# ucuapps/OpenGlue

Hardware: NVIDIA H100
Metric: image-pairs/sec at N=M=2048, d=256, 9 GNN layers, 100 Sinkhorn iters (higher is better)
Workload: dtype fp16x3 (fp16 hi/lo operands with power-of-two tensor scales, 3 products, fp32 accumulate)

## Files before the change

openglue_b200/csrc/sinkhorn.cuh:

```cuda
#pragma once
#include "common.cuh"
#include "tc_common.cuh"
#include <math_constants.h>
#include <algorithm>

namespace og {

struct SinkArgs {
  static constexpr bool kBackward = false;
  const float* S; int64_t lds, strideS;
  const float* dustbin;
  int B, n, m, iters;
  float reg;
  float norm, log_a_last, log_b_last;
  float* scores;
  float* u;
  float* partial;
  unsigned int* barrier;
  int SP, rows_per_strip, mpad;
  float* hist_u;
  float* hist_v;
};

constexpr int SINK_WARPS = 8;
constexpr int64_t SINK_BARRIER_BYTES = 256 * 128;
constexpr int SINK_MAX_COLS = 8192;
constexpr int SINK_MAX_STRIPS = 32;
constexpr float LOG2E_F = 1.4426950408889634f;

__device__ __forceinline__ void grid_barrier(unsigned int* counter, unsigned int target) {
  __syncthreads();
  if (threadIdx.x == 0) {
    __threadfence();
    atomicAdd(counter, 1u);
    unsigned int seen;
    do {
      asm volatile("ld.acquire.gpu.global.u32 %0, [%1];" : "=r"(seen) : "l"(counter) : "memory");
    } while (seen < target);
    __threadfence();
  }
  __syncthreads();
}

typedef unsigned long long f32x2;
__device__ __forceinline__ f32x2 pk2(float x, float y) { f32x2 r; asm("mov.b64 %0, {%1, %2};" : "=l"(r) : "f"(x), "f"(y)); return r; }
__device__ __forceinline__ void upk2(f32x2 v, float& x, float& y) { asm("mov.b64 {%0, %1}, %2;" : "=f"(x), "=f"(y) : "l"(v)); }
#define OG_F32X2_OP(name, expr)                                        \
  __device__ __forceinline__ f32x2 name(f32x2 a, f32x2 b) {            \
    float ax, ay, bx, by; upk2(a, ax, ay); upk2(b, bx, by);            \
    auto op = [](float u, float v) { return expr; };                   \
    return pk2(op(ax, bx), op(ay, by));                                \
  }
OG_F32X2_OP(add2, __fadd_rn(u, v))
OG_F32X2_OP(sub2, __fsub_rn(u, v))
OG_F32X2_OP(mul2, __fmul_rn(u, v))
#undef OG_F32X2_OP
__device__ __forceinline__ f32x2 fma2(f32x2 a, f32x2 b, f32x2 c) {
  float ax, ay, bx, by, cx, cy; upk2(a, ax, ay); upk2(b, bx, by); upk2(c, cx, cy);
  return pk2(__fmaf_rn(ax, bx, cx), __fmaf_rn(ay, by, cy));
}

template <int V, int W>
struct SinkStrip {
  static constexpr int C = 128 * V, MC = W * C, G = SINK_WARPS / W;
  int b, strip, tid, lane, grp, sub, c0, r0, r1;
  template <class Args>
  __device__ __forceinline__ explicit SinkStrip(const Args& a) {
    b = blockIdx.x / a.SP; strip = blockIdx.x % a.SP;
    tid = threadIdx.x; lane = tid & 31;
    grp = (tid >> 5) / W; sub = (tid >> 5) % W;
    c0 = sub * C;
    r0 = strip * a.rows_per_strip;
    r1 = min(r0 + a.rows_per_strip, a.n + 1);
  }
};

template <int V, int W, int SLOTS, bool EVICT_FIRST, class Args>
struct SinkRowRing {
  static constexpr int C = 128 * V, G = SINK_WARPS / W;
  float* slot;
// ... 52 lines not shown
      for (int k = 0; k < V; ++k) z[k] = make_float4(dz, dz, dz, dz);
      return;
    }
    if (!bytes) {
#pragma unroll
      for (int k = 0; k < V; ++k) z[k] = make_float4(0.f, 0.f, 0.f, 0.f);
      return;
    }
    const uint32_t sl = consumed % SLOTS, ph = (consumed / SLOTS) & 1;
    while (!tc::mbar_try_wait(&bar[sl], ph)) {}
    const float4* src = reinterpret_cast<const float4*>(slot + sl * C);
    if (full) {
#pragma unroll
      for (int k = 0; k < V; ++k) z[k] = src[lane + 32 * k];
    } else {
#pragma unroll
      for (int k = 0; k < V; ++k) {
        const int idx = lane + 32 * k;
        const int c = c0 + 4 * idx;
        const int m = a.m;
        float4 q = (c < m) ? src[idx] : make_float4(0.f, 0.f, 0.f, 0.f);
        if (c < m && c + 3 >= m) {
          if (c + 1 >= m) q.y = 0.f;
          if (c + 2 >= m) q.z = 0.f;
          q.w = 0.f;
        }
        z[k] = q;
      }
    }
    ++consumed;
    __syncwarp();
    const int nxt = row + SLOTS * G;
    if (lane == 0 && nxt < end_real) copy(sl, nxt);
    if (a.reg != 1.0f) {
      const float reg = a.reg;
#pragma unroll
      for (int k = 0; k < V; ++k) {
        z[k].x = __fdiv_rn(z[k].x, reg); z[k].y = __fdiv_rn(z[k].y, reg);
        z[k].z = __fdiv_rn(z[k].z, reg); z[k].w = __fdiv_rn(z[k].w, reg);
      }
    }
  }
};

template <int V, int W, class X>
__device__ __forceinline__ const X* sink_row_exchange(X* xr, X mine, const SinkStrip<V, W>& s, uint32_t& rowpar) {
  X* x = xr + (rowpar * SinkStrip<V, W>::G + s.grp) * W;
  if (s.lane == 0) x[s.sub] = mine;
  asm volatile("bar.sync %0, %1;" ::"r"(1 + s.grp), "n"(W * 32) : "memory");
  rowpar ^= 1u;
  return x;
}

template <int V, int W, class Args, class Update>
__device__ __forceinline__ void sink_column_reduce(const Args& a, const SinkStrip<V, W>& s, float* red, const float4 (&cacc)[V],
                                                   float cacc_m, int k, Update update) {
  const int m = a.m;
  float* myred = red + s.grp * a.mpad;
#pragma unroll
  for (int q = 0; q < V; ++q) {
    const int c = s.c0 + 4 * (s.lane + 32 * q);
    if (c < m) *reinterpret_cast<float4*>(myred + c) = cacc[q];
  }
  __syncthreads();
  if (s.sub == 0 && s.lane == 0) myred[m] = cacc_m;
  __syncthreads();
  const int64_t buf = (int64_t)(k & 1) * a.B * a.SP + (int64_t)s.b * a.SP;
  float* part = a.partial + (buf + s.strip) * a.mpad;
  for (int j = s.tid; j <= m; j += blockDim.x) {
    float sum = 0.f;
#pragma unroll
    for (int w = 0; w < SinkStrip<V, W>::G; ++w) sum += red[w * a.mpad + j];
    part[j] = sum;
  }
  grid_barrier(a.barrier + 32 * s.b, (unsigned int)(k + 1) * (unsigned int)a.SP);
  const float* pb = a.partial + buf * a.mpad;
  for (int j4 = s.tid; 4 * j4 <= m; j4 += blockDim.x) {
    float4 c = make_float4(0.f, 0.f, 0.f, 0.f);
#pragma unroll 8
    for (int sp = 0; sp < a.SP; ++sp) {
      const float4 q = __ldcg(reinterpret_cast<const float4*>(pb + (int64_t)sp * a.mpad) + j4);
      c.x += q.x; c.y += q.y; c.z += q.z; c.w += q.w;
    }
    const float cc[4] = {c.x, c.y, c.z, c.w};
#pragma unroll
    for (int e = 0; e < 4; ++e) {
      const int j = 4 * j4 + e;
      if (j < m) update(j, cc[e]);
      else if (j == m) update(SinkStrip<V, W>::MC, cc[e]);
    }
  }
  __syncthreads();
}

template <int V, int W, int SLOTS>
__global__ void __launch_bounds__(SINK_WARPS * 32, (V <= 8) ? 2 : 1) sinkhorn_kernel(SinkArgs a) {
  extern __shared__ __align__(128) float og_sink_smem[];
  using Strip = SinkStrip<V, W>;
  constexpr int C = Strip::C, MC = Strip::MC, G = Strip::G;
  float* v_s = og_sink_smem;
  float* red = og_sink_smem + MC + 4;
  float* ring = red + G * a.mpad;
  uint64_t* bars = reinterpret_cast<uint64_t*>(ring + SINK_WARPS * SLOTS * C);
  float2* xr = reinterpret_cast<float2*>(bars + SINK_WARPS * SLOTS);
  const Strip s(a);
  const int n = a.n, m = a.m, c0 = s.c0, lane = s.lane, sub = s.sub;
  const float a_reg = expf(a.norm), a_last = expf(a.log_a_last);
  SinkRowRing<V, W, SLOTS, true, SinkArgs> rows(a, s, ring, bars);
  const float dz = rows.dz;

  for (int j = s.tid; j < MC; j += blockDim.x) v_s[j] = (j < m) ? 0.f : -CUDART_INF_F;
  if (s.tid == 0) v_s[MC] = 0.f;
  __syncthreads();

  rows.prime();
  uint32_t rowpar = 0;
  const f32x2 log2e2 = pk2(LOG2E_F, LOG2E_F);
  for (int it = 0; it < a.iters; ++it) {
    f32x2 cacc[2 * V];
#pragma unroll
    for (int k = 0; k < 2 * V; ++k) cacc[k] = 0ull;
    float cacc_m = 0.f;
    const float v_m = v_s[MC];

    for (int row = s.r0 + s.grp; row < s.r1; row += G) {
      float4 q[V];
      rows.take(row, q);
      f32x2 z[2 * V];
#pragma unroll
      for (int k = 0; k < V; ++k) { z[2 * k] = pk2(q[k].x, q[k].y); z[2 * k + 1] = pk2(q[k].z, q[k].w); }
      const float t_m = dz + v_m;
      float mx = (sub == 0) ? t_m : -CUDART_INF_F;
#pragma unroll
      for (int k = 0; k < V; ++k) {
        const ulonglong2 vv = *reinterpret_cast<const ulonglong2*>(v_s + c0 + 4 * (lane + 32 * k));
        z[2 * k] = add2(z[2 * k], vv.x); z[2 * k + 1] = add2(z[2 * k + 1], vv.y);
// ... 25 lines not shown
        f_w = ex2_approx((mx - mxg) * LOG2E_F);
      }
      const float w_i = __fdiv_rn((row < n) ? a_reg : a_last, s_i) * f_w;
      if ((it == a.iters - 1 || a.hist_u) && sub == 0 && lane == 0) {
        const float u_i = ((row < n) ? a.norm : a.log_a_last) - (mxg + logf(s_i));
        if (it == a.iters - 1) a.u[(int64_t)s.b * (n + 1) + row] = u_i;
        if (a.hist_u) a.hist_u[((int64_t)s.b * a.iters + it) * (n + 1) + row] = u_i;
      }
      const f32x2 w2 = pk2(w_i, w_i);
#pragma unroll
      for (int k = 0; k < 2 * V; ++k) cacc[k] = fma2(z[k], w2, cacc[k]);
      cacc_m = fmaf(e_m, w_i, cacc_m);
    }
    rows.prime();
    float4 c4[V];
#pragma unroll
    for (int k = 0; k < V; ++k) { upk2(cacc[2 * k], c4[k].x, c4[k].y); upk2(cacc[2 * k + 1], c4[k].z, c4[k].w); }
    sink_column_reduce(a, s, red, c4, cacc_m, it, [&](int j, float c) {
      v_s[j] = ((j < MC) ? a.norm : a.log_b_last) + v_s[j] - logf(c);
    });
    if (a.hist_v && s.strip == 0) {
      float* hv = a.hist_v + ((int64_t)s.b * (a.iters + 1) + it + 1) * (m + 1);
      for (int j = s.tid; j <= m; j += blockDim.x) hv[j] = (j < m) ? v_s[j] : v_s[MC];
    }
  }

  {
    const float v_m = v_s[MC];
    for (int row = s.r0 + s.grp; row < s.r1; row += G) {
      float4 z[V];
      rows.take(row, z);
      float u_i = 0.f;
      if (a.iters > 0) {
        if (lane == 0) u_i = __ldcg(a.u + (int64_t)s.b * (n + 1) + row);
        u_i = __shfl_sync(0xffffffffu, u_i, 0);
      }
      float* out = a.scores + ((int64_t)s.b * (n + 1) + row) * (m + 1);
#pragma unroll
      for (int k = 0; k < V; ++k) {
        const int c = c0 + 4 * (lane + 32 * k);
        if (c < m) {
          const float4 vv = *reinterpret_cast<const float4*>(v_s + c);
          if (c + 0 < m) out[c + 0] = (z[k].x + u_i) + vv.x - a.norm;
          if (c + 1 < m) out[c + 1] = (z[k].y + u_i) + vv.y - a.norm;
          if (c + 2 < m) out[c + 2] = (z[k].z + u_i) + vv.z - a.norm;
          if (c + 3 < m) out[c + 3] = (z[k].w + u_i) + vv.w - a.norm;
        }
      }
      if (sub == 0 && lane == 0) out[m] = (dz + u_i) + v_m - a.norm;
    }
  }
}

struct SinkPlan { int V, W, slots, occ, SP, rows_per_strip, mpad, pairs_per_launch; size_t smem; };

constexpr size_t sinkhorn_smem(bool backward, int V, int W, int slots, int mpad) {
  const int C = 128 * V, G = SINK_WARPS / W, vecs = backward ? 3 : 1;
  const size_t xbytes = backward ? sizeof(float) : sizeof(float2);
  return ((size_t)vecs * (W * C + 4) + (size_t)G * mpad + (size_t)SINK_WARPS * slots * C) * sizeof(float) +
         (size_t)SINK_WARPS * slots * sizeof(uint64_t) + (size_t)2 * G * W * xbytes + 128;
}

inline int sinkhorn_plan(bool backward, int B, int n, int m, SinkPlan* p) {
  const char* who = backward ? "sinkhorn_bwd" : "sinkhorn";
  if (m <= 512)                { p->V = 4;  p->W = 1; p->slots = 2; }
  else if (m <= 1024)          { p->V = 4;  p->W = 2; p->slots = 2; }
  else if (m <= 2048)          { p->V = 8;  p->W = 2; p->slots = 2; }
  else if (m <= 4096)          { p->V = 16; p->W = 2; p->slots = backward ? 1 : 2; }
  else if (m <= SINK_MAX_COLS) { p->V = 16; p->W = 4; p->slots = 1; }
  else return fail(OG_EUNSUPPORTED, "%s: m = %d > %d columns not supported (swap the images)", who, m, SINK_MAX_COLS);
  p->mpad = (int)align_up(m + 1, 4);
  p->smem = sinkhorn_smem(backward, p->V, p->W, p->slots, p->mpad);
  p->occ = (p->V <= 8 && 2 * (p->smem + 1024) <= OG_SMEM_OPTIN_MAX) ? 2 : 1;
  const int sms = device_info().ok ? device_info().sm_count : 132;
  const int ctas = sms * p->occ;
  p->pairs_per_launch = std::min(B < ctas ? B : ctas, (int)(SINK_BARRIER_BYTES / 128));
  int sp = std::min(ctas / p->pairs_per_launch, SINK_MAX_STRIPS);
  const int max_sp = cdiv(n + 1, SINK_WARPS / p->W);
  if (sp > max_sp) sp = max_sp;
  if (sp < 1) sp = 1;
  p->SP = sp;
  p->rows_per_strip = cdiv(n + 1, sp);
  return OG_OK;
}

inline int sinkhorn_check_rows(const char* who, const float* S, int64_t lds, int64_t strideS, int m) {
  if (lds % 4 != 0 || lds < m || (reinterpret_cast<uintptr_t>(S) & 15) || strideS % 4 != 0)
    return fail(OG_EINVAL, "%s: S rows must be 16-byte aligned (lds %% 4 == 0, lds >= m)", who);
  return OG_OK;
}

struct SinkConsts { float norm, log_a_last, log_b_last; };
inline SinkConsts sinkhorn_consts(int n, int m) {
  const float norm = -logf((float)(n + m));
  return {norm, norm + (float)log((double)m),
          norm + (float)log((double)n)};
}

template <auto Kernel, int V, int W, int SLOTS, class Args>
inline int sinkhorn_coop_launch(const Args& a, const SinkPlan& p, cudaStream_t stream) {
  constexpr size_t smem_max = sinkhorn_smem(Args::kBackward, V, W, SLOTS, 128 * V * W + 4);
  static_assert(smem_max <= OG_SMEM_OPTIN_MAX, "Sinkhorn kernel: shared memory beyond what one block may opt in to");
  if (const int rc = smem_opt_in<Kernel>((int)smem_max)) return rc;
  cudaLaunchConfig_t cfg = {};
  cfg.gridDim = dim3(a.B * a.SP);
  cfg.blockDim = dim3(SINK_WARPS * 32);
  cfg.dynamicSmemBytes = p.smem;
  cfg.stream = stream;
  cudaLaunchAttribute attr[1];
  attr[0].id = cudaLaunchAttributeCooperative;
  attr[0].val.cooperative = 1;
  cfg.attrs = attr; cfg.numAttrs = 1;
  OG_CUDA(cudaLaunchKernelEx(&cfg, Kernel, a));
  launch_counter()++;
  return OG_OK;
}

template <class Launch>
inline int sinkhorn_for_each_launch(const SinkPlan& p, int B, unsigned int* barrier, cudaStream_t stream, Launch&& launch) {
  for (int b0 = 0; b0 < B; b0 += p.pairs_per_launch) {
    const int nb = std::min(p.pairs_per_launch, B - b0);
    OG_CUDA(cudaMemsetAsync(barrier, 0, (size_t)nb * 128, stream));
    if (const int rc = launch(b0, nb)) return rc;
  }
  return OG_OK;
}

inline int64_t sinkhorn_workspace_bytes(int B, int n, int m) {
  SinkPlan p;
  if (sinkhorn_plan(false, B, n, m, &p) != OG_OK) return -1;
  return SINK_BARRIER_BYTES + align_up((int64_t)B * (n + 1) * 4, 256) + align_up(2LL * B * SINK_MAX_STRIPS * p.mpad * 4, 256);
}

inline int sinkhorn_launch(const float* S, int64_t lds, int64_t strideS, const float* dustbin, int B, int n, int m,
                           int iters, float reg, float* scores, void* ws, int64_t ws_bytes, cudaStream_t stream,
                           float* hist_u = nullptr, float* hist_v = nullptr) {
  SinkPlan p;
  if (const int rc = sinkhorn_plan(false, B, n, m, &p)) return rc;
  if (ws_bytes < sinkhorn_workspace_bytes(B, n, m)) return fail(OG_EWORKSPACE, "sinkhorn: workspace too small");
  if (const int rc = sinkhorn_check_rows("sinkhorn", S, lds, strideS, m)) return rc;
  char* w = static_cast<char*>(ws);
  unsigned int* barrier = reinterpret_cast<unsigned int*>(w); w += SINK_BARRIER_BYTES;
  float* u = reinterpret_cast<float*>(w); w += align_up((int64_t)B * (n + 1) * 4, 256);
  float* partial = reinterpret_cast<float*>(w);
  const SinkConsts k = sinkhorn_consts(n, m);
  if (hist_v) OG_CUDA(cudaMemsetAsync(hist_v, 0, (size_t)B * (iters + 1) * (m + 1) * sizeof(float), stream));
  return sinkhorn_for_each_launch(p, B, barrier, stream, [&](int b0, int nb) {
    SinkArgs a;
    a.S = S + (int64_t)b0 * strideS; a.lds = lds; a.strideS = strideS; a.dustbin = dustbin;
    a.B = nb; a.n = n; a.m = m; a.iters = iters; a.reg = reg;
    a.norm = k.norm; a.log_a_last = k.log_a_last; a.log_b_last = k.log_b_last;
    a.scores = scores + (int64_t)b0 * (n + 1) * (m + 1);
    a.u = u; a.partial = partial; a.barrier = barrier;
    a.SP = p.SP; a.rows_per_strip = p.rows_per_strip; a.mpad = p.mpad;
    a.hist_u = hist_u ? hist_u + (int64_t)b0 * iters * (n + 1) : nullptr;
    a.hist_v = hist_v ? hist_v + (int64_t)b0 * (iters + 1) * (m + 1) : nullptr;
    if (p.V == 4 && p.W == 1) return sinkhorn_coop_launch<sinkhorn_kernel<4, 1, 2>, 4, 1, 2>(a, p, stream);
    if (p.V == 4)             return sinkhorn_coop_launch<sinkhorn_kernel<4, 2, 2>, 4, 2, 2>(a, p, stream);
    if (p.V == 8)             return sinkhorn_coop_launch<sinkhorn_kernel<8, 2, 2>, 8, 2, 2>(a, p, stream);
    if (p.W == 2)             return sinkhorn_coop_launch<sinkhorn_kernel<16, 2, 2>, 16, 2, 2>(a, p, stream);
    return sinkhorn_coop_launch<sinkhorn_kernel<16, 4, 1>, 16, 4, 1>(a, p, stream);
  });
}

}
```

openglue_b200/csrc/sinkhorn_bwd.cuh:

```cuda
#pragma once
#include "sinkhorn.cuh"

namespace og {

struct SinkBwdArgs {
  static constexpr bool kBackward = true;
  const float* S; int64_t lds, strideS;
  const float* dustbin;
  int B, n, m, iters;
  float reg, norm, log_a_last, log_b_last;
  const float* hist_u;
  const float* hist_v;
  const float* ubar_init;
  const float* vbar_init;
  float* hist_coef;
  float* hist_cvec;
  float* hist_vbar;
  float* hist_wq;
  float* partial;
  unsigned int* barrier;
  int SP, rows_per_strip, mpad;
};

template <int V, int W, int SLOTS>
__global__ void __launch_bounds__(SINK_WARPS * 32, (V <= 8) ? 2 : 1) sinkhorn_bwd_kernel(SinkBwdArgs a) {
  extern __shared__ __align__(128) float og_sinkb_smem[];
  using Strip = SinkStrip<V, W>;
  constexpr int C = Strip::C, MC = Strip::MC, G = Strip::G;
  float* cvec_s = og_sinkb_smem;
  float* vbar_s = cvec_s + MC + 4;
  float* wq_s = vbar_s + MC + 4;
  float* red = wq_s + MC + 4;
  float* ring = red + G * a.mpad;
  uint64_t* bars = reinterpret_cast<uint64_t*>(ring + SINK_WARPS * SLOTS * C);
  float* xr = reinterpret_cast<float*>(bars + SINK_WARPS * SLOTS);
  const Strip s(a);
  const int n = a.n, m = a.m, T = a.iters, b = s.b, tid = s.tid;
  const float ia_reg = expf(-a.norm), ia_last = expf(-a.log_a_last);
  SinkRowRing<V, W, SLOTS, false, SinkBwdArgs> rows(a, s, ring, bars);
  const float dz = rows.dz;

  for (int j = tid; j <= MC; j += blockDim.x) {
    float vb = 0.f;
    if (j < m) vb = __ldg(a.vbar_init + (int64_t)b * (m + 1) + j);
    else if (j == MC) vb = __ldg(a.vbar_init + (int64_t)b * (m + 1) + m);
    vbar_s[j] = vb;
  }
  __syncthreads();

  rows.prime();
  uint32_t rowpar = 0;
  for (int it = T - 1; it >= 0; --it) {
    const float* vt = a.hist_v + ((int64_t)b * (T + 1) + it + 1) * (m + 1);
    const float* vtm1 = vt - (m + 1);
    for (int j = tid; j <= MC; j += blockDim.x) {
      float cv = -CUDART_INF_F, wq = 0.f;
      const int jj = (j < m) ? j : (j == MC ? m : -1);
      if (jj >= 0) {
        const float lb = (jj < m) ? a.norm : a.log_b_last;
        cv = __ldcg(vt + jj) - lb;
        wq = expf(__ldcg(vtm1 + jj) - cv);
      }
      cvec_s[j] = cv; wq_s[j] = wq;
    }
    __syncthreads();
    if (s.strip == 0) {
      const int64_t o = ((int64_t)b * T + it) * (m + 1);
      for (int j = tid; j <= m; j += blockDim.x) {
        const int js = (j < m) ? j : MC;
        a.hist_cvec[o + j] = cvec_s[js]; a.hist_vbar[o + j] = vbar_s[js]; a.hist_wq[o + j] = wq_s[js];
      }
    }
    float4 cacc[V];
#pragma unroll
// ... 159 lines not shown

inline int64_t sinkhorn_hist_floats(int B, int n, int m, int T) { return (int64_t)B * T * (n + 1) + (int64_t)B * (T + 1) * (m + 1); }

inline int64_t sinkhorn_bwd_workspace_bytes(int B, int n, int m, int T) {
  SinkPlan p;
  if (sinkhorn_plan(true, B, n, m, &p) != OG_OK) return -1;
  const int64_t nrs = cdiv(n + 1, SINKB_RS_ROWS);
  int64_t f = 0;
  f += align_up((int64_t)B * (n + 1), 64) + align_up((int64_t)B * (m + 1), 64);
  f += align_up((int64_t)B * nrs * (m + 1), 64);
  f += align_up((int64_t)B * T * (n + 1), 64) + 3 * align_up((int64_t)B * T * (m + 1), 64);
  f += align_up(2LL * B * SINK_MAX_STRIPS * p.mpad, 64) + align_up((int64_t)B, 64);
  return SINK_BARRIER_BYTES + 256 + f * 4;
}

inline int sinkhorn_bwd_launch(const float* S, int64_t lds, int64_t strideS, const float* dustbin, int B, int n, int m, int iters, float reg,
                               const float* hist, const float* G, float* dZ, float* ddustbin, void* ws, int64_t ws_bytes,
                               cudaStream_t stream) {
  SinkPlan p;
  if (const int rc = sinkhorn_plan(true, B, n, m, &p)) return rc;
  if (ws_bytes < sinkhorn_bwd_workspace_bytes(B, n, m, iters)) return fail(OG_EWORKSPACE, "sinkhorn_bwd: workspace too small");
  if (const int rc = sinkhorn_check_rows("sinkhorn_bwd", S, lds, strideS, m)) return rc;
  const int T = iters;
  const int64_t nrs = cdiv(n + 1, SINKB_RS_ROWS);
  char* w = static_cast<char*>(ws);
  unsigned int* barrier = reinterpret_cast<unsigned int*>(w); w += SINK_BARRIER_BYTES;
  unsigned int* counter = reinterpret_cast<unsigned int*>(w); w += 256;
  float* f = reinterpret_cast<float*>(w);
  auto take = [&](int64_t nfl) { float* r = f; f += align_up(nfl, 64); return r; };
  float* ubar_init = take((int64_t)B * (n + 1));
  float* vbar_init = take((int64_t)B * (m + 1));
  float* colpart = take((int64_t)B * nrs * (m + 1));
  float* hist_coef = take((int64_t)B * T * (n + 1));
  float* hist_cvec = take((int64_t)B * T * (m + 1));
  float* hist_vbar = take((int64_t)B * T * (m + 1));
  float* hist_wq = take((int64_t)B * T * (m + 1));
  float* partial = take(2LL * B * SINK_MAX_STRIPS * p.mpad);
  float* per_pair = take(B);
  const SinkConsts k = sinkhorn_consts(n, m);
  const int m1 = m + 1, n1 = n + 1;
  sinkb_rowsum_kernel<<<cdiv(B * n1, 8), 256, 0, stream>>>(G, B * n1, m1, ubar_init);
  OG_LAUNCH_CHECK("sinkb_rowsum_kernel");
  sinkb_colsum_kernel<<<dim3(cdiv(m1, 256), (unsigned)nrs, B), 256, 0, stream>>>(G, n1, m1, colpart);
  OG_LAUNCH_CHECK("sinkb_colsum_kernel");
  sinkb_colsum_finish_kernel<<<dim3(cdiv(m1, 256), B), 256, 0, stream>>>(colpart, (int)nrs, m1, vbar_init);
  OG_LAUNCH_CHECK("sinkb_colsum_finish_kernel");
  launch_counter() += 3;
  SinkBwdArgs a;
  a.S = S; a.lds = lds; a.strideS = strideS; a.dustbin = dustbin; a.B = B; a.n = n; a.m = m; a.iters = T; a.reg = reg;
  a.norm = k.norm; a.log_a_last = k.log_a_last; a.log_b_last = k.log_b_last;
  a.hist_u = hist; a.hist_v = hist + (int64_t)B * T * (n + 1);
  a.ubar_init = ubar_init; a.vbar_init = vbar_init;
  a.hist_coef = hist_coef; a.hist_cvec = hist_cvec; a.hist_vbar = hist_vbar; a.hist_wq = hist_wq;
  a.partial = partial; a.barrier = barrier; a.SP = p.SP; a.rows_per_strip = p.rows_per_strip; a.mpad = p.mpad;
  if (T > 0) {
    const int rc = sinkhorn_for_each_launch(p, B, barrier, stream, [&](int b0, int nb) {
      SinkBwdArgs g = a;
      g.B = nb;
      g.S = S + (int64_t)b0 * strideS;
      g.hist_u = a.hist_u + (int64_t)b0 * T * n1; g.hist_v = a.hist_v + (int64_t)b0 * (T + 1) * m1;
      g.ubar_init = ubar_init + (int64_t)b0 * n1; g.vbar_init = vbar_init + (int64_t)b0 * m1;
      g.hist_coef = hist_coef + (int64_t)b0 * T * n1; g.hist_cvec = hist_cvec + (int64_t)b0 * T * m1;
      g.hist_vbar = hist_vbar + (int64_t)b0 * T * m1; g.hist_wq = hist_wq + (int64_t)b0 * T * m1;
      if (p.V == 4 && p.W == 1) return sinkhorn_coop_launch<sinkhorn_bwd_kernel<4, 1, 2>, 4, 1, 2>(g, p, stream);
      if (p.V == 4)             return sinkhorn_coop_launch<sinkhorn_bwd_kernel<4, 2, 2>, 4, 2, 2>(g, p, stream);
      if (p.V == 8)             return sinkhorn_coop_launch<sinkhorn_bwd_kernel<8, 2, 2>, 8, 2, 2>(g, p, stream);
      if (p.W == 2)             return sinkhorn_coop_launch<sinkhorn_bwd_kernel<16, 2, 1>, 16, 2, 1>(g, p, stream);
      return sinkhorn_coop_launch<sinkhorn_bwd_kernel<16, 4, 1>, 16, 4, 1>(g, p, stream);
    });
    if (rc != OG_OK) return rc;
  }
  sinkb_dz_kernel<<<dim3(cdiv(m1, SINKB_TC), cdiv(n1, SINKB_TR), B), 256, 0, stream>>>(a, G, dZ, 1.f / reg);
  OG_LAUNCH_CHECK("sinkb_dz_kernel");
  OG_CUDA(cudaMemsetAsync(counter, 0, 4, stream));
  sinkb_dustbin_kernel<<<B, 256, 0, stream>>>(dZ, B, n, m, per_pair, counter, ddustbin);
  OG_LAUNCH_CHECK("sinkb_dustbin_kernel");
  launch_counter() += 2;
  return OG_OK;
}

}
```

openglue_b200/csrc/linear_sm90.cuh:

```cuda
#pragma once
#include "tc_common.cuh"
#include <algorithm>
#include <type_traits>

namespace og {

struct TcLinearArgs {
  const float* A;  int64_t lda;  int64_t strideA;
  const float* A2; int64_t lda2; int64_t strideA2;
  int k1, k2;
  int b_rows_per_batch;
  const float* bias;
  int rows, nout, batch;
  float alpha;
  int relu;
  const float* R; int64_t ldr; int64_t strideR;
  const float* rscale;
  float* Y;   float* Yhi;  float* Ylo;  int64_t ldy;  int64_t strideY;
  float* Yt;  float* Ythi; float* Ytlo; int64_t ldyt; int64_t strideYt;
};

struct F16LinearArgs {
  const float* A;  int64_t lda;  int64_t strideA;
  const float* A2; int64_t lda2; int64_t strideA2;
// ... 125 lines not shown
      if (*timeout_flag) asm volatile("trap;");
    }
    return;
  }
  setmaxnreg_inc<240>();
  const int c = wg - 1, tid = threadIdx.x & 127, warp = tid >> 5, lane = tid & 31, g = lane >> 2, t = lane & 3;
  const int r0 = c * 64 + warp * 16 + g;

  float s_a = 1.f, amax_a = 0.f;
  if constexpr (F16) {
#pragma unroll
    for (int i = 0; i < 3; ++i) if (a.amax_in[i]) amax_a = fmaxf(amax_a, __ldcg(a.amax_in[i]));
    s_a = f16_scale_for(amax_a);
    if (blockIdx.x == 0 && threadIdx.x == 128) {
      if (a.nkinds > 1) {
        for (int kk = 0; kk < a.nkinds; ++kk) {
          const float* w2 = a.w_meta + 4 * kk;
          const float so = f16_scale_for(fabsf(a.alpha) * fmaf(amax_a, __ldg(w2 + 1), __ldg(w2 + 2)));
          if (a.kind0 + kk == 1 && a.scale_out) *a.scale_out = so;
          if (a.kind0 + kk == 2 && a.scale_out_v) *a.scale_out_v = so;
        }
      } else if (!a.Y && a.scale_out) {
        *a.scale_out = f16_scale_for(fabsf(a.alpha) * fmaf(amax_a, __ldg(a.w_meta + 1), __ldg(a.w_meta + 2)));
      }
    }
  }

  float racc[64], acc[64];
  uint32_t ahi0[4][4], alo0[4][4], ahi1[4][4], alo1[4][4];
  uint32_t it = 0, timed_out = 0;

  auto split_a = [&](uint32_t it_, uint32_t (&ahi)[4][4], uint32_t (&alo)[4][4]) {
    const int s = it_ % S;
    mbar_wait_flag(&full[s], (it_ / S) & 1, timed_out);
    const uint8_t* st = smem + s * C::STAGE;
#pragma unroll
    for (int kk = 0; kk < 4; ++kk) {
      if constexpr (F16) {
        const uint8_t* box = st + (kk >> 1) * BM * 128;
        const int col = (kk & 1) * 16 + 2 * t;
#pragma unroll
        for (int q = 0; q < 4; ++q) {
          const float2 v = *reinterpret_cast<const float2*>(sw128_f32(box, r0 + (q & 1) * 8, col + (q >> 1) * 8));
          split_f16x2(v.x * s_a, v.y * s_a, ahi[kk][q], alo[kk][q]);
          if (a.swap_halves) { ahi[kk][q] = __byte_perm(ahi[kk][q], 0, 0x1032); alo[kk][q] = __byte_perm(alo[kk][q], 0, 0x1032); }
        }
      } else {
#pragma unroll
        for (int q = 0; q < 4; ++q) split_tf32(*sw128_f32(st, r0 + (q & 1) * 8, 8 * kk + t + (q >> 1) * 4), ahi[kk][q], alo[kk][q]);
      }
    }
  };

  if (c == 1) named_bar_arrive(TURN + 0, 256);
#pragma unroll 1
  for (int tile = blockIdx.x; tile < ntiles; tile += gridDim.x) {
    int n0, m0, bz;
    tile_origin(tile, tiles_n, tiles_m, n0, m0, bz);
    const bool last_tile = tile + (int)gridDim.x >= ntiles;
#pragma unroll
    for (int i = 0; i < 64; ++i) racc[i] = 0.f;

    auto mma_block = [&](int kb, const uint32_t (&ahi)[4][4], const uint32_t (&alo)[4][4], uint32_t (&nhi)[4][4],
                         uint32_t (&nlo)[4][4]) {
      const int s = it % S;
      const bool last = last_tile && kb == nkb - 1;
      if (last && timed_out) *timeout_flag = 1;
      const uint32_t bhi = smem_u32(smem + s * C::STAGE + C::A_BYTES), blo = bhi + C::B_TILE;
      named_bar_sync(TURN + c, 256);
      fence_operands(acc);
      wgmma_fence();
#pragma unroll
      for (int kk = 0; kk < 4; ++kk) {
        const uint64_t dhi = make_wgdesc_sw128(bhi + kk * 32), dlo = make_wgdesc_sw128(blo + kk * 32);
        const int acc0 = (kb % C::CHUNK != 0 || kk) ? 1 : 0;
        if constexpr (F16) {
          wgmma_f16_m64n128(acc, alo[kk], dhi, acc0);
          wgmma_f16_m64n128(acc, ahi[kk], dlo, 1);
          wgmma_f16_m64n128(acc, ahi[kk], dhi, 1);
        } else {
          wgmma_tf32_m64n128(acc, alo[kk], dhi, acc0);
          wgmma_tf32_m64n128(acc, ahi[kk], dlo, 1);
          wgmma_tf32_m64n128(acc, ahi[kk], dhi, 1);
        }
      }
      wgmma_commit();
      if (!(last && c == 1)) named_bar_arrive(TURN + (c ^ 1), 256);
      if (kb + 1 < nkb) split_a(it + 1, nhi, nlo);
      wgmma_wait<0>();
      fence_operands(acc);
      if (tid == 0) mbar_arrive(&empty[s]);
      if (kb % C::CHUNK == C::CHUNK - 1 || kb == nkb - 1) {
#pragma unroll
        for (int i = 0; i < 64; ++i) racc[i] += acc[i];
      }
      ++it;
    };
    split_a(it, ahi0, alo0);
#pragma unroll 1
    for (int kb = 0; kb < nkb; kb += 2) {
      mma_block(kb, ahi0, alo0, ahi1, alo1);
      if (kb + 1 < nkb) mma_block(kb + 1, ahi1, alo1, ahi0, alo0);
    }

    if constexpr (F16) {
      const float s_w = __ldg(a.w_meta);
      int okind = a.Y ? 1 : (a.Yh ? 2 : 3), kidx = 0, ocols = a.nout;
      float alpha_t = a.alpha / (s_a * s_w), sos = 1.f;
      const float* wm = a.w_meta;
      if (a.nkinds > 1) {
        kidx = n0 / a.kind_cols; okind = a.kind0 + kidx + 1; ocols = a.kind_cols;
        wm = a.w_meta + 4 * kidx;
        alpha_t = a.alpha / (s_a * __ldg(wm));
      }
      if (okind != 1) sos = f16_scale_for(fabsf(a.alpha) * fmaf(amax_a, __ldg(wm + 1), __ldg(wm + 2)));
      float tmax = 0.f;
      if (okind == 1) {
#pragma unroll
        for (int h = 0; h < 2; ++h) {
          const int grow = m0 + r0 + 8 * h;
          if (grow >= a.rows) continue;
          const float* rrow = a.R ? a.R + (int64_t)bz * a.strideR + (int64_t)grow * a.ldr : nullptr;
#pragma unroll
          for (int jh = 0; jh < 16; jh += 8) {
            float bv[16], rv[16];
#pragma unroll
            for (int i = 0; i < 16; ++i) {
              const int col = n0 + 8 * (jh + (i >> 1)) + 2 * t + (i & 1);
              const bool in = col < a.nout;
              bv[i] = a.bias && in ? __ldg(a.bias + col) : 0.f;
              rv[i] = rrow && in ? rrow[col] : 0.f;
            }
#pragma unroll
            for (int jj = 0; jj < 8; ++jj) {
              const int j = jh + jj;
              const int col = n0 + 8 * j + 2 * t;
              if (col >= a.nout) continue;
              const bool two = col + 1 < a.nout;
              float y0 = fmaf(racc[4 * j + 2 * h], alpha_t, bv[2 * jj]);
              float y1 = two ? fmaf(racc[4 * j + 2 * h + 1], alpha_t, bv[2 * jj + 1]) : 0.f;
              if (a.relu) { y0 = fmaxf(y0, 0.f); y1 = fmaxf(y1, 0.f); }
              const int64_t o = (int64_t)bz * a.strideY + (int64_t)grow * a.ldy + col;
              if (a.R) {
                y0 += rv[2 * jj];
                if (two) y1 += rv[2 * jj + 1];
              }
              if (two) *reinterpret_cast<float2*>(a.Y + o) = make_float2(y0, y1);
              else a.Y[o] = y0;
              tmax = fmaxf(tmax, fmaxf(fabsf(y0), fabsf(y1)));
            }
          }
        }
      } else {
        uint32_t hv[2][16], lv[2][16];
#pragma unroll
        for (int j = 0; j < 16; ++j) {
          const int col = n0 + 8 * j + 2 * t;
          const bool two = col + 1 < a.nout;
          const float b0 = a.bias && col < a.nout ? __ldg(a.bias + col) : 0.f;
          const float b1 = a.bias && two ? __ldg(a.bias + col + 1) : 0.f;
#pragma unroll
          for (int h = 0; h < 2; ++h) {
            float y0 = fmaf(racc[4 * j + 2 * h], alpha_t, b0);
            float y1 = two ? fmaf(racc[4 * j + 2 * h + 1], alpha_t, b1) : 0.f;
            if (a.relu) { y0 = fmaxf(y0, 0.f); y1 = fmaxf(y1, 0.f); }
            split_f16x2(y0 * sos, y1 * sos, hv[h][j], lv[h][j]);
          }
        }
        if (okind == 2) {
          const bool wide = a.ldy % 8 == 0 && a.strideY % 8 == 0 && al16(a.Yh) && al16(a.Yl);
#pragma unroll
          for (int h = 0; h < 2; ++h) {
            const int grow = m0 + r0 + 8 * h;
            const int64_t orow = (int64_t)bz * a.strideY + (int64_t)grow * a.ldy - kidx * ocols;
            if (wide) {
#pragma unroll
              for (int q = 0; q < 4; ++q) {
                const uint4 vh = quad_gather_b16(hv[h], q, t), vl = quad_gather_b16(lv[h], q, t);
                const int col = n0 + 8 * (4 * q + t);
                if (grow >= a.rows || col >= a.nout) continue;
                if (col + 8 <= a.nout) {
                  *reinterpret_cast<uint4*>(a.Yh + orow + col) = vh;
                  *reinterpret_cast<uint4*>(a.Yl + orow + col) = vl;
                } else {
                  store_b16_run(a.Yh + orow + col, vh, a.nout - col);
                  store_b16_run(a.Yl + orow + col, vl, a.nout - col);
                }
              }
            } else if (grow < a.rows) {
#pragma unroll
              for (int j = 0; j < 16; ++j) {
                const int col = n0 + 8 * j + 2 * t;
                if (col >= a.nout) continue;
                store_half_pair(a.Yh + orow + col, hv[h][j], col + 1 < a.nout);
                store_half_pair(a.Yl + orow + col, lv[h][j], col + 1 < a.nout);
              }
            }
          }
        } else {
#pragma unroll
          for (int h = 0; h < 2; ++h) {
            const int grow = m0 + r0 + 8 * h;
            if (grow < a.rows) {
#pragma unroll
              for (int j = 0; j < 16; ++j) {
                const int col = n0 + 8 * j + 2 * t;
// ... 5 lines not shown
                  a.Ytl[o + a.ldyt] = __ushort_as_half((unsigned short)(lv[h][j] >> 16));
                }
              }
            }
          }
        }
      }
      if (okind == 1 && a.amax_out) {
        tmax = warp_max(tmax);
        if (lane == 0 && tmax > 0.f) atomic_amax(a.amax_out, tmax);
      }
    } else {
#pragma unroll
      for (int h = 0; h < 2; ++h) {
        const int grow = m0 + r0 + 8 * h;
        if (grow >= a.rows) continue;
        const float* rrow = a.R ? a.R + (int64_t)bz * a.strideR + (int64_t)grow * a.ldr : nullptr;
        const int64_t yoff = (int64_t)bz * a.strideY + (int64_t)grow * a.ldy;
        const int64_t ytoff = (int64_t)bz * a.strideYt + grow;
#pragma unroll
        for (int jh = 0; jh < 16; jh += 8) {
          float bv[16], sv[16], rv[16];
#pragma unroll
          for (int i = 0; i < 16; ++i) {
            const int col = n0 + 8 * (jh + (i >> 1)) + 2 * t + (i & 1);
            const bool in = col < a.nout;
            bv[i] = a.bias && in ? __ldg(a.bias + col) : 0.f;
            sv[i] = rrow && a.rscale && in ? __ldg(a.rscale + col) : 0.f;
            rv[i] = rrow && in ? rrow[col] : 0.f;
          }
#pragma unroll
          for (int jj = 0; jj < 8; ++jj) {
            const int j = jh + jj;
#pragma unroll
            for (int e = 0; e < 2; ++e) {
              const int col = n0 + 8 * j + 2 * t + e;
              if (col >= a.nout) continue;
              float v = racc[4 * j + 2 * h + e] * a.alpha;
              if (a.bias) v += bv[2 * jj + e];
              if (a.relu) v = fmaxf(v, 0.f);
              if (rrow) { const float r = rv[2 * jj + e]; v = a.rscale ? fmaf(sv[2 * jj + e], r, v) : (v + r); }
              uint32_t vh = 0, vl = 0;
              if (a.Yhi || a.Ythi) split_tf32(v, vh, vl);
              if (a.Y) a.Y[yoff + col] = v;
              if (a.Yhi) { a.Yhi[yoff + col] = __uint_as_float(vh); a.Ylo[yoff + col] = __uint_as_float(vl); }
              const int64_t o = ytoff + (int64_t)col * a.ldyt;
              if (a.Yt) a.Yt[o] = v;
              if (a.Ythi) { a.Ythi[o] = __uint_as_float(vh); a.Ytlo[o] = __uint_as_float(vl); }
            }
          }
        }
      }
    }
  }
}

template <class Args, class BT>
inline int linear_sm90_launch(const Args& a, const BT* Bhi, const BT* Blo, int64_t ldb, int64_t b_total_rows, cudaStream_t stream) {
  using namespace tcf;
  constexpr bool F16 = std::is_same<Args, F16LinearArgs>::value;
  using C = Cfg<F16>;
  const int K = a.k1 + a.k2;
  CUtensorMap ma, ma2, mh, ml;
  int rc;
  if ((rc = tc::make_tmap_3d(&ma, a.A, a.strideA ? a.batch : 1, a.rows, a.k1, a.lda, a.strideA, BM)) != OG_OK) return rc;
  if (a.A2) { if ((rc = tc::make_tmap_3d(&ma2, a.A2, a.strideA2 ? a.batch : 1, a.rows, a.k2, a.lda2, a.strideA2, BM)) != OG_OK) return rc; }
  else ma2 = ma;
  if constexpr (F16) {
    if ((rc = tc::make_tmap_2d_f16(&mh, Bhi, (uint64_t)b_total_rows, (uint64_t)K, (uint64_t)ldb, BN)) != OG_OK) return rc;
    if ((rc = tc::make_tmap_2d_f16(&ml, Blo, (uint64_t)b_total_rows, (uint64_t)K, (uint64_t)ldb, BN)) != OG_OK) return rc;
  } else {
    if ((rc = tc::make_tmap_2d(&mh, Bhi, (uint64_t)b_total_rows, (uint64_t)K, (uint64_t)ldb, BN)) != OG_OK) return rc;
    if ((rc = tc::make_tmap_2d(&ml, Blo, (uint64_t)b_total_rows, (uint64_t)K, (uint64_t)ldb, BN)) != OG_OK) return rc;
  }
  if ((rc = smem_opt_in<linear_sm90_kernel<Args>>(C::SMEM_BYTES)) != OG_OK) return rc;
  const int tiles = cdiv(a.nout, BN) * cdiv(a.rows, BM) * a.batch;
  const int sms = device_info().ok ? device_info().sm_count : 132;
  return tc::pdl_launch(linear_sm90_kernel<Args>, dim3(std::min(tiles, sms)), dim3(THREADS), C::SMEM_BYTES, stream, ma, ma2, mh, ml, a);
}
template int linear_sm90_launch(const TcLinearArgs&, const float*, const float*, int64_t, int64_t, cudaStream_t);
template int linear_sm90_launch(const F16LinearArgs&, const __half*, const __half*, int64_t, int64_t, cudaStream_t);

inline bool linear_sm90_eligible(const TcLinearArgs& a, const float* Bhi, const float* Blo, int64_t ldb) {
  const int K = a.k1 + a.k2;
  return K >= 32 && a.k1 % 4 == 0 && a.k2 % 4 == 0 && a.lda % 4 == 0 && a.strideA % 4 == 0 && al16(a.A) &&
         (!a.A2 || (a.k1 % 32 == 0 && a.lda2 % 4 == 0 && a.strideA2 % 4 == 0 && al16(a.A2))) && ldb % 4 == 0 && al16(Bhi) && al16(Blo);
}

inline bool linear_sm90_eligible(const F16LinearArgs& a, const __half* Bh, const __half* Bl, int64_t ldb) {
  const int K = a.k1 + a.k2;
  if (!(K >= 64 && a.k1 % 4 == 0 && a.k2 % 4 == 0 && a.lda % 4 == 0 && a.strideA % 4 == 0 && al16(a.A) && ldb % 8 == 0 && al16(Bh) && al16(Bl))) return false;
  if (a.A2 && (a.k1 % 32 != 0 || a.lda2 % 4 != 0 || a.strideA2 % 4 != 0 || !al16(a.A2))) return false;
  if (!a.w_meta || !(a.amax_in[0] || a.amax_in[1] || a.amax_in[2])) return false;
  const int kinds = (a.Y ? 1 : 0) + (a.Yh ? 1 : 0) + (a.Yth ? 1 : 0);
  if (a.nkinds > 1) {
    if (a.kind0 < 0 || a.kind0 + a.nkinds > 3 || kinds != a.nkinds || a.kind_cols % tcf::BN != 0 || a.nout != a.nkinds * a.kind_cols) return false;
    if ((a.kind0 == 0) != (a.Y != nullptr) || !a.Yh || (a.kind0 + a.nkinds == 3) != (a.Yth != nullptr) || a.R || a.relu) return false;
    if (a.Yth && !a.scale_out_v) return false;
  } else if (kinds != 1) return false;
  if (a.Y && !(a.ldy % 2 == 0 && a.strideY % 2 == 0 && al16(a.Y))) return false;
  if (a.Yh && !(a.Yl && a.ldy % 2 == 0 && a.strideY % 2 == 0 && al16(a.Yh) && al16(a.Yl) && !a.R && a.scale_out)) return false;
  if (a.Yth && !(a.Ytl && !a.R && (a.scale_out || a.scale_out_v))) return false;
  return true;
}

__global__ void __launch_bounds__(256) split_tf32_kernel(const float* __restrict__ src, float* __restrict__ hi,
// ... 40 lines not shown
```

Before: 440.8.

## Allow more Sinkhorn row strips with a two-phase scattered column reduction

For the forward Sinkhorn, the strip count per pair may now exceed 32, up to the SM count, as long as each strip keeps at least 16 rows. With that many strips, each CTA reduces only its own slice of columns across all strip partials, writes the result to a colsum buffer, and a second grid barrier follows before every CTA reads the full column sums. The goal is to use more SMs when the batch is small and to stop every CTA from re-reading all SP partial rows. The cost is an extra grid barrier per iteration and a larger workspace.

```diff
diff --git a/openglue_b200/csrc/sinkhorn.cuh b/openglue_b200/csrc/sinkhorn.cuh
--- a/openglue_b200/csrc/sinkhorn.cuh
+++ b/openglue_b200/csrc/sinkhorn.cuh
@@ -16,8 +16,10 @@
   float* scores;
   float* u;
   float* partial;
+  float* colsum;
   unsigned int* barrier;
   int SP, rows_per_strip, mpad;
+  bool scatter;
   float* hist_u;
   float* hist_v;
 };
@@ -26,6 +28,7 @@
 constexpr int64_t SINK_BARRIER_BYTES = 256 * 128;
 constexpr int SINK_MAX_COLS = 8192;
 constexpr int SINK_MAX_STRIPS = 32;
+constexpr int SINK_MIN_STRIP_ROWS = 16;
 constexpr float LOG2E_F = 1.4426950408889634f;
 
 __device__ __forceinline__ void grid_barrier(unsigned int* counter, unsigned int target) {
@@ -184,6 +187,12 @@
   return x;
 }
 
+__device__ __forceinline__ float4 ldcg_ordered(const float4* p) {
+  float4 r;
+  asm volatile("ld.global.cg.v4.f32 {%0, %1, %2, %3}, [%4];" : "=f"(r.x), "=f"(r.y), "=f"(r.z), "=f"(r.w) : "l"(p));
+  return r;
+}
+
 template <int V, int W, class Args, class Update>
 __device__ __forceinline__ void sink_column_reduce(const Args& a, const SinkStrip<V, W>& s, float* red, const float4 (&cacc)[V],
                                                    float cacc_m, int k, Update update) {
@@ -205,15 +214,48 @@
     for (int w = 0; w < SinkStrip<V, W>::G; ++w) sum += red[w * a.mpad + j];
     part[j] = sum;
   }
-  grid_barrier(a.barrier + 32 * s.b, (unsigned int)(k + 1) * (unsigned int)a.SP);
+  unsigned int* const bar = a.barrier + 32 * s.b;
   const float* pb = a.partial + buf * a.mpad;
-  for (int j4 = s.tid; 4 * j4 <= m; j4 += blockDim.x) {
+  auto strip_sum = [&](int j4) {
     float4 c = make_float4(0.f, 0.f, 0.f, 0.f);
 #pragma unroll 8
     for (int sp = 0; sp < a.SP; ++sp) {
-      const float4 q = __ldcg(reinterpret_cast<const float4*>(pb + (int64_t)sp * a.mpad) + j4);
+      const float4 q = ldcg_ordered(reinterpret_cast<const float4*>(pb + (int64_t)sp * a.mpad) + j4);
       c.x += q.x; c.y += q.y; c.z += q.z; c.w += q.w;
     }
+    return c;
+  };
+  float4* const colsum = reinterpret_cast<float4*>(a.colsum + (int64_t)s.b * a.mpad);
+  if (a.scatter) {
+    grid_barrier(bar, (unsigned int)(2 * k + 1) * (unsigned int)a.SP);
+    const int n4 = a.mpad / 4, per = cdiv(n4, a.SP), j0 = s.strip * per, cols = max(0, min(per, n4 - j0));
+    const int nch = cdiv(a.SP, SINK_MAX_STRIPS);
+    float4* const chunk = reinterpret_cast<float4*>(red);
+    for (int i = s.tid; i < nch * cols; i += blockDim.x) {
+      const int ch = i / cols, j4 = j0 + i % cols, sp1 = min((ch + 1) * SINK_MAX_STRIPS, a.SP);
+      float4 t = make_float4(0.f, 0.f, 0.f, 0.f);
+#pragma unroll 8
+      for (int sp = ch * SINK_MAX_STRIPS; sp < sp1; ++sp) {
+        const float4 q = ldcg_ordered(reinterpret_cast<const float4*>(pb + (int64_t)sp * a.mpad) + j4);
+        t.x += q.x; t.y += q.y; t.z += q.z; t.w += q.w;
+      }
+      chunk[i] = t;
+    }
+    __syncthreads();
+    for (int jj = s.tid; jj < cols; jj += blockDim.x) {
+      float4 c = make_float4(0.f, 0.f, 0.f, 0.f);
+      for (int ch = 0; ch < nch; ++ch) {
+        const float4 t = chunk[ch * cols + jj];
+        c.x += t.x; c.y += t.y; c.z += t.z; c.w += t.w;
+      }
+      __stcg(colsum + j0 + jj, c);
+    }
+    grid_barrier(bar, (unsigned int)(2 * k + 2) * (unsigned int)a.SP);
+  } else {
+    grid_barrier(bar, (unsigned int)(k + 1) * (unsigned int)a.SP);
+  }
+  for (int j4 = s.tid; 4 * j4 <= m; j4 += blockDim.x) {
+    const float4 c = a.scatter ? ldcg_ordered(colsum + j4) : strip_sum(j4);
     const float cc[4] = {c.x, c.y, c.z, c.w};
 #pragma unroll
     for (int e = 0; e < 4; ++e) {
@@ -345,7 +387,7 @@
   }
 }
 
-struct SinkPlan { int V, W, slots, occ, SP, rows_per_strip, mpad, pairs_per_launch; size_t smem; };
+struct SinkPlan { int V, W, slots, occ, SP, rows_per_strip, mpad, pairs_per_launch; size_t smem; bool scatter; };
 
 constexpr size_t sinkhorn_smem(bool backward, int V, int W, int slots, int mpad) {
   const int C = 128 * V, G = SINK_WARPS / W, vecs = backward ? 3 : 1;
@@ -368,12 +410,14 @@
   const int sms = device_info().ok ? device_info().sm_count : 132;
   const int ctas = sms * p->occ;
   p->pairs_per_launch = std::min(B < ctas ? B : ctas, (int)(SINK_BARRIER_BYTES / 128));
-  int sp = std::min(ctas / p->pairs_per_launch, SINK_MAX_STRIPS);
+  const int cap = backward ? SINK_MAX_STRIPS : std::max(SINK_MAX_STRIPS, std::min(sms, (n + 1) / SINK_MIN_STRIP_ROWS));
+  int sp = std::min(ctas / p->pairs_per_launch, cap);
   const int max_sp = cdiv(n + 1, SINK_WARPS / p->W);
   if (sp > max_sp) sp = max_sp;
   if (sp < 1) sp = 1;
   p->SP = sp;
   p->rows_per_strip = cdiv(n + 1, sp);
+  p->scatter = sp > SINK_MAX_STRIPS;
   return OG_OK;
 }
 
@@ -419,10 +463,12 @@
   return OG_OK;
 }
 
+inline int64_t sinkhorn_reduce_floats(const SinkPlan& p) { return (int64_t)p.pairs_per_launch * (2LL * p.SP + 1) * p.mpad; }
+
 inline int64_t sinkhorn_workspace_bytes(int B, int n, int m) {
   SinkPlan p;
   if (sinkhorn_plan(false, B, n, m, &p) != OG_OK) return -1;
-  return SINK_BARRIER_BYTES + align_up((int64_t)B * (n + 1) * 4, 256) + align_up(2LL * B * SINK_MAX_STRIPS * p.mpad * 4, 256);
+  return SINK_BARRIER_BYTES + align_up((int64_t)B * (n + 1) * 4, 256) + align_up(sinkhorn_reduce_floats(p) * 4, 256);
 }
 
 inline int sinkhorn_launch(const float* S, int64_t lds, int64_t strideS, const float* dustbin, int B, int n, int m,
@@ -444,8 +490,8 @@
     a.B = nb; a.n = n; a.m = m; a.iters = iters; a.reg = reg;
     a.norm = k.norm; a.log_a_last = k.log_a_last; a.log_b_last = k.log_b_last;
     a.scores = scores + (int64_t)b0 * (n + 1) * (m + 1);
-    a.u = u; a.partial = partial; a.barrier = barrier;
-    a.SP = p.SP; a.rows_per_strip = p.rows_per_strip; a.mpad = p.mpad;
+    a.u = u; a.partial = partial; a.colsum = partial + 2LL * p.pairs_per_launch * p.SP * p.mpad; a.barrier = barrier;
+    a.SP = p.SP; a.rows_per_strip = p.rows_per_strip; a.mpad = p.mpad; a.scatter = p.scatter;
     a.hist_u = hist_u ? hist_u + (int64_t)b0 * iters * (n + 1) : nullptr;
     a.hist_v = hist_v ? hist_v + (int64_t)b0 * (iters + 1) * (m + 1) : nullptr;
     if (p.V == 4 && p.W == 1) return sinkhorn_coop_launch<sinkhorn_kernel<4, 1, 2>, 4, 1, 2>(a, p, stream);
diff --git a/openglue_b200/csrc/sinkhorn_bwd.cuh b/openglue_b200/csrc/sinkhorn_bwd.cuh
--- a/openglue_b200/csrc/sinkhorn_bwd.cuh
+++ b/openglue_b200/csrc/sinkhorn_bwd.cuh
@@ -18,8 +18,10 @@
   float* hist_vbar;
   float* hist_wq;
   float* partial;
+  float* colsum;
   unsigned int* barrier;
   int SP, rows_per_strip, mpad;
+  bool scatter;
 };
 
 template <int V, int W, int SLOTS>
@@ -285,7 +287,8 @@
   a.hist_u = hist; a.hist_v = hist + (int64_t)B * T * (n + 1);
   a.ubar_init = ubar_init; a.vbar_init = vbar_init;
   a.hist_coef = hist_coef; a.hist_cvec = hist_cvec; a.hist_vbar = hist_vbar; a.hist_wq = hist_wq;
-  a.partial = partial; a.barrier = barrier; a.SP = p.SP; a.rows_per_strip = p.rows_per_strip; a.mpad = p.mpad;
+  a.partial = partial; a.colsum = nullptr; a.scatter = p.scatter;
+  a.barrier = barrier; a.SP = p.SP; a.rows_per_strip = p.rows_per_strip; a.mpad = p.mpad;
   if (T > 0) {
     const int rc = sinkhorn_for_each_launch(p, B, barrier, stream, [&](int b0, int nb) {
       SinkBwdArgs g = a;
```

Result: no change. 439.8 (median of 6 runs) (-0.2%).

## Defer fp32 output epilogue into next tile's first MMA block

Applied to the files above, without the earlier changes.

For fp16x3 linear tiles that write plain fp32 Y with no residual, the epilogue is postponed and run inside the next tile's first k-block, after its wgmma batch is issued, so the global stores overlap tensor-core work. Instead of zeroing the accumulator at tile start, the first chunk now overwrites it, which keeps the deferred tile's values alive until they are stored. The fp32 epilogue loop is also restructured to load bias and residual values for both row halves per column group, in smaller groups when deferred. The deferred epilogue competes for registers with the in-flight MMA and the next A split, which adds register pressure.

```diff
diff --git a/openglue_b200/csrc/linear_sm90.cuh b/openglue_b200/csrc/linear_sm90.cuh
--- a/openglue_b200/csrc/linear_sm90.cuh
+++ b/openglue_b200/csrc/linear_sm90.cuh
@@ -201,57 +201,9 @@
     }
   };
 
-  if (c == 1) named_bar_arrive(TURN + 0, 256);
-#pragma unroll 1
-  for (int tile = blockIdx.x; tile < ntiles; tile += gridDim.x) {
+  auto epilogue = [&](int tile, auto only_y) {
     int n0, m0, bz;
     tile_origin(tile, tiles_n, tiles_m, n0, m0, bz);
-    const bool last_tile = tile + (int)gridDim.x >= ntiles;
-#pragma unroll
-    for (int i = 0; i < 64; ++i) racc[i] = 0.f;
-
-    auto mma_block = [&](int kb, const uint32_t (&ahi)[4][4], const uint32_t (&alo)[4][4], uint32_t (&nhi)[4][4],
-                         uint32_t (&nlo)[4][4]) {
-      const int s = it % S;
-      const bool last = last_tile && kb == nkb - 1;
-      if (last && timed_out) *timeout_flag = 1;
-      const uint32_t bhi = smem_u32(smem + s * C::STAGE + C::A_BYTES), blo = bhi + C::B_TILE;
-      named_bar_sync(TURN + c, 256);
-      fence_operands(acc);
-      wgmma_fence();
-#pragma unroll
-      for (int kk = 0; kk < 4; ++kk) {
-        const uint64_t dhi = make_wgdesc_sw128(bhi + kk * 32), dlo = make_wgdesc_sw128(blo + kk * 32);
-        const int acc0 = (kb % C::CHUNK != 0 || kk) ? 1 : 0;
-        if constexpr (F16) {
-          wgmma_f16_m64n128(acc, alo[kk], dhi, acc0);
-          wgmma_f16_m64n128(acc, ahi[kk], dlo, 1);
-          wgmma_f16_m64n128(acc, ahi[kk], dhi, 1);
-        } else {
-          wgmma_tf32_m64n128(acc, alo[kk], dhi, acc0);
-          wgmma_tf32_m64n128(acc, ahi[kk], dlo, 1);
-          wgmma_tf32_m64n128(acc, ahi[kk], dhi, 1);
-        }
-      }
-      wgmma_commit();
-      if (!(last && c == 1)) named_bar_arrive(TURN + (c ^ 1), 256);
-      if (kb + 1 < nkb) split_a(it + 1, nhi, nlo);
-      wgmma_wait<0>();
-      fence_operands(acc);
-      if (tid == 0) mbar_arrive(&empty[s]);
-      if (kb % C::CHUNK == C::CHUNK - 1 || kb == nkb - 1) {
-#pragma unroll
-        for (int i = 0; i < 64; ++i) racc[i] += acc[i];
-      }
-      ++it;
-    };
-    split_a(it, ahi0, alo0);
-#pragma unroll 1
-    for (int kb = 0; kb < nkb; kb += 2) {
-      mma_block(kb, ahi0, alo0, ahi1, alo1);
-      if (kb + 1 < nkb) mma_block(kb + 1, ahi1, alo1, ahi0, alo0);
-    }
-
     if constexpr (F16) {
       const float s_w = __ldg(a.w_meta);
       int okind = a.Y ? 1 : (a.Yh ? 2 : 3), kidx = 0, ocols = a.nout;
@@ -265,23 +217,27 @@
       if (okind != 1) sos = f16_scale_for(fabsf(a.alpha) * fmaf(amax_a, __ldg(wm + 1), __ldg(wm + 2)));
       float tmax = 0.f;
       if (okind == 1) {
-#pragma unroll
-        for (int h = 0; h < 2; ++h) {
-          const int grow = m0 + r0 + 8 * h;
-          if (grow >= a.rows) continue;
-          const float* rrow = a.R ? a.R + (int64_t)bz * a.strideR + (int64_t)grow * a.ldr : nullptr;
-#pragma unroll
-          for (int jh = 0; jh < 16; jh += 8) {
-            float bv[16], rv[16];
-#pragma unroll
-            for (int i = 0; i < 16; ++i) {
-              const int col = n0 + 8 * (jh + (i >> 1)) + 2 * t + (i & 1);
-              const bool in = col < a.nout;
-              bv[i] = a.bias && in ? __ldg(a.bias + col) : 0.f;
-              rv[i] = rrow && in ? rrow[col] : 0.f;
-            }
-#pragma unroll
-            for (int jj = 0; jj < 8; ++jj) {
+        constexpr int JB = decltype(only_y)::value ? 2 : 4;
+        const bool in0 = m0 + r0 < a.rows, in1 = m0 + r0 + 8 < a.rows;
+        const float* rrow0 = a.R && in0 ? a.R + (int64_t)bz * a.strideR + (int64_t)(m0 + r0) * a.ldr : nullptr;
+        const float* rrow1 = a.R && in1 ? a.R + (int64_t)bz * a.strideR + (int64_t)(m0 + r0 + 8) * a.ldr : nullptr;
+#pragma unroll
+        for (int jh = 0; jh < 16; jh += JB) {
+          float bv[2 * JB], rv[2][2 * JB];
+#pragma unroll
+          for (int i = 0; i < 2 * JB; ++i) {
+            const int col = n0 + 8 * (jh + (i >> 1)) + 2 * t + (i & 1);
+            const bool in = col < a.nout;
+            bv[i] = a.bias && in ? a.bias[col] : 0.f;
+            rv[0][i] = rrow0 && in ? rrow0[col] : 0.f;
+            rv[1][i] = rrow1 && in ? rrow1[col] : 0.f;
+          }
+#pragma unroll
+          for (int h = 0; h < 2; ++h) {
+            const int grow = m0 + r0 + 8 * h;
+            if (grow >= a.rows) continue;
+#pragma unroll
+            for (int jj = 0; jj < JB; ++jj) {
               const int j = jh + jj;
               const int col = n0 + 8 * j + 2 * t;
               if (col >= a.nout) continue;
@@ -291,8 +247,8 @@
               if (a.relu) { y0 = fmaxf(y0, 0.f); y1 = fmaxf(y1, 0.f); }
               const int64_t o = (int64_t)bz * a.strideY + (int64_t)grow * a.ldy + col;
               if (a.R) {
-                y0 += rv[2 * jj];
-                if (two) y1 += rv[2 * jj + 1];
+                y0 += rv[h][2 * jj];
+                if (two) y1 += rv[h][2 * jj + 1];
               }
               if (two) *reinterpret_cast<float2*>(a.Y + o) = make_float2(y0, y1);
               else a.Y[o] = y0;
@@ -300,7 +256,7 @@
             }
           }
         }
-      } else {
+      } else if constexpr (!decltype(only_y)::value) {
         uint32_t hv[2][16], lv[2][16];
 #pragma unroll
         for (int j = 0; j < 16; ++j) {
@@ -412,6 +368,76 @@
         }
       }
     }
+  };
+  auto y_tile = [&](int n0) -> bool {
+    if constexpr (F16) return !a.R && (a.nkinds > 1 ? a.kind0 + n0 / a.kind_cols + 1 : (a.Y ? 1 : (a.Yh ? 2 : 3))) == 1;
+    else return false;
+  };
+
+  if (c == 1) named_bar_arrive(TURN + 0, 256);
+  int pending = -1;
+#pragma unroll 1
+  for (int tile = blockIdx.x; tile < ntiles; tile += gridDim.x) {
+    int n0, m0, bz;
+    tile_origin(tile, tiles_n, tiles_m, n0, m0, bz);
+    const bool last_tile = tile + (int)gridDim.x >= ntiles;
+
+#pragma unroll
+    for (int i = 0; i < 64; ++i) if constexpr (!F16) racc[i] = 0.f;
+
+    auto mma_block = [&](int kb, const uint32_t (&ahi)[4][4], const uint32_t (&alo)[4][4], uint32_t (&nhi)[4][4],
+                         uint32_t (&nlo)[4][4], auto defer) {
+      const int s = it % S;
+      const bool last = last_tile && kb == nkb - 1;
+      if (last && timed_out) *timeout_flag = 1;
+      const uint32_t bhi = smem_u32(smem + s * C::STAGE + C::A_BYTES), blo = bhi + C::B_TILE;
+      named_bar_sync(TURN + c, 256);
+      fence_operands(acc);
+      wgmma_fence();
+#pragma unroll
+      for (int kk = 0; kk < 4; ++kk) {
+        const uint64_t dhi = make_wgdesc_sw128(bhi + kk * 32), dlo = make_wgdesc_sw128(blo + kk * 32);
+        const int acc0 = (kb % C::CHUNK != 0 || kk) ? 1 : 0;
+        if constexpr (F16) {
+          wgmma_f16_m64n128(acc, alo[kk], dhi, acc0);
+          wgmma_f16_m64n128(acc, ahi[kk], dlo, 1);
+          wgmma_f16_m64n128(acc, ahi[kk], dhi, 1);
+        } else {
+          wgmma_tf32_m64n128(acc, alo[kk], dhi, acc0);
+          wgmma_tf32_m64n128(acc, ahi[kk], dlo, 1);
+          wgmma_tf32_m64n128(acc, ahi[kk], dhi, 1);
+        }
+      }
+      wgmma_commit();
+      if (!(last && c == 1)) named_bar_arrive(TURN + (c ^ 1), 256);
+      if constexpr (decltype(defer)::value) {
+        if (kb == 0 && pending >= 0) epilogue(pending, std::true_type());
+      }
+      if (kb + 1 < nkb) split_a(it + 1, nhi, nlo);
+      wgmma_wait<0>();
+      fence_operands(acc);
+      if (tid == 0) mbar_arrive(&empty[s]);
+      if (kb % C::CHUNK == C::CHUNK - 1 || kb == nkb - 1) {
+#pragma unroll
+        for (int i = 0; i < 64; ++i) {
+          if constexpr (F16) racc[i] = kb < C::CHUNK ? __fadd_rn(0.f, acc[i]) : racc[i] + acc[i];
+          else racc[i] += acc[i];
+        }
+      }
+      ++it;
+    };
+    split_a(it, ahi0, alo0);
+#pragma unroll 1
+    for (int kb = 0; kb < nkb; kb += 2) {
+      mma_block(kb, ahi0, alo0, ahi1, alo1, std::bool_constant<F16>());
+      if (kb + 1 < nkb) mma_block(kb + 1, ahi1, alo1, ahi0, alo0, std::false_type());
+    }
+    pending = -1;
+    if (y_tile(n0)) pending = tile;
+    else epilogue(tile, std::false_type());
+  }
+  if constexpr (F16) {
+    if (pending >= 0) epilogue(pending, std::true_type());
   }
 }
 
```

After: 332.1 before, 334.7 after (median of 6 runs). Within noise of the previous version (+0.8%).
